# degleris1/CMF.jl

Measured on AMD Instinct MI355X. Metric: MU iters/sec (convolutive NMF multiplicative update; achieved HBM GB/s in `hbm`), higher is better.
Workload: dtype f32

## Files before the change

### cmf.jl_amd/csrc/cmf_api.hip

```cpp
#include "cmf_internal.h"

static void wb_free(cmf_handle_s *h);
static void wb_disarm(cmf_handle_s *h);

size_t n_partial(const cmf_handle_s *h)
{
    const CmfDims &d = h->d;
    size_t n = (size_t)(64 * h->conv_gx) * (size_t)std::max(h->conv_gy, h->conv_gy_ext);
    n = std::max(n, (size_t)(d.Np / 64) * d.KB * d.L);
    n = std::max(n, (size_t)((d.Tl + 63) / 64) * d.KB);
    n = std::max(n, 2 * (((size_t)d.Tl * d.K32 + 1023) / 1024));
    return n;
}

static int ensure_stage(cmf_handle_s *h, size_t elems)
{
    if (h->stage_elems >= elems) return CMF_OK;
    if (h->stage) HIPCHK(hipFree(h->stage));
    h->stage = nullptr;
    h->stage_elems = 0;
    HIPCHK(hipMalloc(&h->stage, elems * sizeof(double)));
    h->stage_elems = elems;
    return CMF_OK;
}
// ... 354 lines not shown
    const CmfDims &d = h->d;
    h->spec_gen = -1;
    HxtParams p;
    p.H = h->H; p.X0 = X0; p.X1 = X1; p.slabs = slabs;
    p.Np = NpX; p.K32 = d.K32; p.KB = d.KB; p.PADL = d.PADL; p.L = d.L; p.Tl = main_rows >= 0 ? main_rows : d.Tl; p.chunk_len = chunk_len;
    p.G = h->hxt_groups; p.nsrc = nsrc;
    p.CG = hxt_cg(nchunks);
    dim3 grid((NpX / 128) * p.CG * h->hxt_groups, nchunks / p.CG, nsrc * d.KB), block(256);
    switch (h->hxt_LP) {
#define CASE(LP_) case LP_: hipLaunchKernelGGL((hxt_kernel<LP_>), grid, block, 0, h->stream, p); break;
        CASE(1) CASE(2) CASE(3) CASE(4) CASE(5) CASE(6) CASE(8)
#undef CASE
    default: return fail(CMF_ERR_STATE, "internal: bad hxt LP %d", h->hxt_LP);
    }
    for (int i = 0; i < 7; ++i)
        if (kHxtLP[i] == h->hxt_LP) h->launches[LA_HXT + i] += 1;
    h->launches[nsrc == 1 ? LA_HXT_NSRC1 : LA_HXT_NSRC2] += 1;
    h->launches[p.Tl < d.Tl ? LA_HXT_TAIL : LA_HXT_NO_TAIL] += 1;
    KCHK("hxt_kernel");
    return CMF_OK;
}

static int launch_hxt(cmf_handle_s *h)
{
    return launch_hxt_on(h, h->X, h->est, h->d.Np, 2, h->wslabs, h->hxt_nchunks, h->hxt_chunk_len, h->hxt_main);
}

int launch_transconv(cmf_handle_s *h, int nsrc, const float *xt0, bool front_block)
{
    if (h->sk_tc) return launch_transconv_small(h, nsrc, xt0);
    ProfScope prof_(h, nsrc == 2 ? PROF_TRANSCONV : PROF_TRANSCONV_1);
    const CmfDims &d = h->d;
    TcParams p;
    p.Wn = h->Wn; p.XT0 = xt0 ? xt0 : h->XT; p.XT1 = h->estT; p.slabs = h->hslabs;
    p.NpW = d.Np;
    p.TP = d.TP; p.PADL = d.PADL; p.K32 = d.K32; p.KB = d.KB; p.L = d.L; p.Tl = d.Tl;
    p.nsrc = nsrc;
    p.C = (int)(rup(d.N, 8) / 8);
    p.W = nsrc == 2 ? h->tc_W : h->tc_W1;
    p.F = nsrc == 2 ? h->tc_S : h->tc_S1;
    p.wtab = h->tc_tab[nsrc == 2 ? 0 : 1];
    p.t_first = 0;
    p.slab_rows = d.Tl;
    if (front_block) {
        p.W = h->tc_W2; p.F = h->tc_S2; p.wtab = h->tc_tab[2];
        p.t_first = -128;
        p.slab_rows = d.Tl + 128;
    }
    dim3 grid((p.W + 3) / 4), block(256);
    switch (h->tc_LT) {
#define CASE(LT_) case LT_: hipLaunchKernelGGL((transconv_kernel<LT_>), grid, block, 0, h->stream, p); break;
        CASE(4) CASE(8) CASE(12) CASE(16) CASE(20) CASE(24) CASE(28) CASE(32)
#undef CASE
    default: return fail(CMF_ERR_STATE, "internal: bad transconv LT %d", h->tc_LT);
    }
    h->launches[LA_TC + h->tc_LT / 4 - 1] += 1;
    if (front_block) h->launches[LA_TC_FRONT] += 1;
    if (p.W >= 64 && p.W % 32 == 0) h->launches[LA_TC_XCD] += 1;
    KCHK("transconv_kernel");
    return CMF_OK;
}

int launch_slab_sum(cmf_handle_s *h, float *out, const float *in, int nslabs, size_t stride, bool take_carry,
                           CmfHxtTail tail)
{
    size_t n4 = stride / 4;
    int blocks = (int)std::min<size_t>(2048, (n4 + 255) / 256);
    CmfLossCarry carry{};
    if (take_carry && h->carry.partial) {
        carry = h->carry;
        h->carry = CmfLossCarry{};
    }
    hipLaunchKernelGGL(slab_sum_kernel, dim3(blocks + (carry.partial ? 1 : 0)), dim3(256), 0, h->stream, out, in, nslabs, stride, n4, carry, tail);
    h->launches[carry.partial ? LA_SLAB_SUM_CARRY : LA_SLAB_SUM] += 1;
    KCHK("slab_sum_kernel");
    return CMF_OK;
}

int hxt_contract(cmf_handle_s *h, const float *X0, const float *X1, int nsrc, float *out, bool take_carry, bool slabs_only)
{
    const CmfDims &d = h->d;
    h->spec_gen = -1;
    if (h->small_k) return hxt_contract_small(h, X0, X1, nsrc, out, take_carry, slabs_only);
    const int nch = nsrc == 2 ? h->hxt_nchunks : h->hxt_nchunks1, clen = nsrc == 2 ? h->hxt_chunk_len : h->hxt_chunk_len1;
    const int main_rows = nsrc == 2 ? h->hxt_main : h->hxt_main1;
    CMFTRY(launch_hxt_on(h, X0, X1, d.Np, nsrc, h->wslabs, nch, clen, main_rows));
    const CmfHxtTail tail{h->H, X0, X1, d.Tl - main_rows, d.PADL + main_rows, d.L, d.K32, d.Np};
    return launch_slab_sum(h, out, h->wslabs, hxt_nslabs(nch), (size_t)nsrc * d.L * d.K32 * d.Np, take_carry, tail);
}

int read_scalar(cmf_handle_s *h, int slot, double *v)
{
    HIPCHK(hipMemcpyAsync(h->h_scalar + slot, h->d_scalar + slot, sizeof(double), hipMemcpyDeviceToHost, h->stream));
    HIPCHK(hipStreamSynchronize(h->stream));
    *v = h->h_scalar[slot];
    return CMF_OK;
}

static int check_ready(cmf_handle_s *h, bool need_data)
{
    if (!h) return fail(CMF_ERR_ARG, "handle is NULL");
    if (h->root_only) return fail(CMF_ERR_STATE, "this entry needs a single-GPU handle, not the front handle of a cmf_create_multi group");
    HIPCHK(hipSetDevice(h->device));
    if (!h->factors_set) return fail(CMF_ERR_STATE, "factors not set: call cmf_set_factors first");
    if (need_data && !h->have_data) return fail(CMF_ERR_STATE, "handle was created without data");
    return CMF_OK;
}

static bool w_speculated(cmf_handle_s *h)
{
    const bool hit = h->spec_gen >= 0 && h->spec_gen == h->est_gen && h->reuse_est && h->est_kind == mu_est_kind(h) && !h->carry.partial;
    h->spec_gen = -1;
    if (hit) h->spec_hits += 1;
    return hit;
}

static int mu_conv_est(cmf_handle_s *h)
{
    return h->mu_mask ? launch_conv<8>(h, h->est, h->d.Tl, h->conv_gy) : launch_conv<0>(h, h->est, h->d.Tl, h->conv_gy);
}

int w_partial_impl(cmf_handle_s *h)
{
    const CmfDims &d = h->d;
    if (w_speculated(h)) return CMF_OK;
    if (!(h->reuse_est && h->est_kind == mu_est_kind(h)))
        CMFTRY(mu_conv_est(h));
    set_est(h, mu_est_kind(h));
    return hxt_contract(h, mu_X(h), h->est, 2, h->numden, true);
}

int w_partial_half_impl(cmf_handle_s *h, int den)
{
    const CmfDims &d = h->d;
    const size_t LKN = (size_t)d.L * d.K32 * d.Np;
    if (den) {
        if (!(h->reuse_est && h->est_kind == 1))
            CMFTRY(launch_conv<0>(h, h->est, d.Tl, h->conv_gy));
        set_est(h, 1);
    }
    const float *src = den ? h->est : h->X;
    return hxt_contract(h, src, src, 1, h->numden + (den ? LKN : 0), den != 0);
}

static int w_apply_impl_(cmf_handle_s *h, double l1W, double l2W, const float *tail_src, float *tail_dst, int tail_n, const float *den);
int w_apply_impl(cmf_handle_s *h, double l1W, double l2W, const float *tail_src, float *tail_dst, int tail_n,
                        const float *den)
{
    return w_apply_impl_(h, l1W, l2W, tail_src, tail_dst, tail_n, den);
}

static int kl_w_phase_impl(cmf_handle_s *h, double l1W, double l2W)
{
    const CmfDims &d = h->d;
    if (h->mu_mask) {
        if (!(h->reuse_est && h->est_kind == 8)) CMFTRY(launch_conv<12>(h, h->est, d.Tl, h->conv_gy, h->Xm));
        set_est(h, 8);
        CMFTRY(hxt_contract(h, h->est, h->M, 2, h->numden, true));
        return w_apply_impl(h, l1W, l2W, nullptr, nullptr, 0, nullptr);
    }
    if (!(h->reuse_est && h->est_kind == 7)) CMFTRY(launch_conv<12>(h, h->est, d.Tl, h->conv_gy));
    set_est(h, 7);
    CMFTRY(hxt_contract(h, h->est, h->est, 1, h->numden, true));
    float *den = h->numden + (size_t)d.L * d.K32 * d.Np;
    hipLaunchKernelGGL(kl_hsum_kernel, dim3(d.K, KL_HCHUNKS), dim3(256), 0, h->stream, h->Ht, d.TP, d.PADL, d.Tl, h->kl_sums);
    KCHK("kl_hsum_kernel");
    hipLaunchKernelGGL(kl_den_w_kernel, dim3(d.L, d.K), dim3(256), 0, h->stream, h->Ht, h->kl_sums, den, d.TP, d.PADL, d.Tl, d.K32, d.Np);
    KCHK("kl_den_w_kernel");
    return w_apply_impl(h, l1W, l2W, nullptr, nullptr, 0, den);
}

static int kl_h_update_impl(cmf_handle_s *h, double l1H, double l2H)
{
    const CmfDims &d = h->d;
    if (h->mu_mask) {
        CMFTRY(launch_conv<13>(h, h->estT, d.Tl + h->halo_r, h->conv_gy_ext, h->XmT));
        CMFTRY(launch_transconv(h, 2, h->MT));
        const size_t TKm = (size_t)d.Tl * d.K32;
        hipLaunchKernelGGL(h_update_kernel, dim3((d.Tl + HUPD_T - 1) / HUPD_T, d.KB), dim3(256), 0, h->stream, h->H, h->Ht, h->hslabs + TKm, 2 * TKm, h->tc_S,
                           h->hslabs, 2 * TKm, h->tc_S, d.Tl, d.K, d.K32, d.PADL, d.TP, (float)l1H, (float)(2.0 * l2H));
        KCHK("h_update_kernel");
        set_est(h, 0);
        return wb_after_H(h);
    }
    CMFTRY(launch_conv<13>(h, h->estT, d.Tl + h->halo_r, h->conv_gy_ext));
    CMFTRY(launch_transconv(h, 1, h->estT));
    hipLaunchKernelGGL(kl_wsum_kernel, dim3(d.L, d.K), dim3(256), 0, h->stream, h->Wt, d.K32, d.Np, h->kl_sums);
    KCHK("kl_wsum_kernel");
    const size_t TK = (size_t)d.Tl * d.K32;
    hipLaunchKernelGGL(kl_den_h_kernel, dim3((unsigned)((TK + 255) / 256)), dim3(256), 0, h->stream, h->kl_sums, h->kl_denH, d.Tl, d.K, d.K32, d.L);
    KCHK("kl_den_h_kernel");
    hipLaunchKernelGGL(h_update_kernel, dim3((d.Tl + HUPD_T - 1) / HUPD_T, d.KB), dim3(256), 0, h->stream, h->H, h->Ht, h->hslabs, TK, h->tc_S1,
                       h->kl_denH, (size_t)0, 1, d.Tl, d.K, d.K32, d.PADL, d.TP, (float)l1H, (float)(2.0 * l2H));
    KCHK("h_update_kernel");
    set_est(h, 0);
    return wb_after_H(h);
}

static int w_phase_impl(cmf_handle_s *h, double l1W, double l2W)
{
    const CmfDims &d = h->d;
    if (h->mu_div) return kl_w_phase_impl(h, l1W, l2W);
    if (!h->small_k) {
        CMFTRY(w_partial_impl(h));
        return w_apply_impl(h, l1W, l2W);
    }
    if (!w_speculated(h)) {
        if (!(h->reuse_est && h->est_kind == mu_est_kind(h)))
            CMFTRY(mu_conv_est(h));
        set_est(h, mu_est_kind(h));
        CMFTRY(hxt_contract(h, mu_X(h), h->est, 2, nullptr, false, true));
    }
    CmfLossCarry carry{};
    if (h->carry.partial) {
        carry = h->carry;
        h->carry = CmfLossCarry{};
    }
    hipLaunchKernelGGL(w_update_small_kernel, dim3(d.Np / 64 + 1, d.L, d.K), dim3(256), 0, h->stream, h->Wt, h->Wn, h->sk_tc ? h->sk_Wj : nullptr, h->sk_slabs,
                       h->sk_ngroups, d.N, d.K, d.L, d.Np, d.K32, h->sk_JP, h->sk3_Kg, h->sk3_GR, h->sk3_JP,
                       (float)l1W, (float)(2.0 * l2W), carry);
    KCHK("w_update_small_kernel");
    set_est(h, 0);
    h->sk_wj_gen = h->sk_tc ? h->est_gen : -1;
    return CMF_OK;
}

static int w_apply_impl_(cmf_handle_s *h, double l1W, double l2W, const float *tail_src, float *tail_dst, int tail_n, const float *den)
{
    const CmfDims &d = h->d;
    dim3 grid(d.Np / 64, d.KB, d.L);
    if (!den) den = h->numden + (size_t)d.L * d.K32 * d.Np;
    hipLaunchKernelGGL(w_update_kernel, grid, dim3(256), 0, h->stream, h->Wt, h->Wn, h->numden, den,
                       d.N, d.K, d.L, d.Np, d.K32, (float)l1W, (float)(2.0 * l2W), tail_src, tail_dst, tail_n);
    KCHK("w_update_kernel");
    set_est(h, 0);
    return CMF_OK;
}

int h_update_impl(cmf_handle_s *h, double l1H, double l2H, bool front)
{
    const CmfDims &d = h->d;
    if (front) {
        if (!h->halo_ext || !h->left_data) return fail(CMF_ERR_STATE, "internal: this shard cannot update the columns in front of its own");
        int np = 0;
        CMFTRY(launch_conv_rows<1>(h, h->estT, -1, 1 + (d.Tl + h->halo_r + 63) / 64, 0, h->n_cu, nullptr, nullptr, nullptr, &np, d.Tl + h->halo_r));
        CMFTRY(launch_transconv(h, 2, nullptr, true));
        const int hx = h->halo_ext, R = d.Tl + 128;
        dim3 gridx((d.Tl + hx + HUPD_T - 1) / HUPD_T, d.KB);
        const float *num = h->hslabs + (size_t)(128 - hx) * d.K32;
        hipLaunchKernelGGL(h_update_kernel, gridx, dim3(256), 0, h->stream, h->H, h->Ht, num, (size_t)2 * R * d.K32, h->tc_S2, num + (size_t)R * d.K32,
                           (size_t)2 * R * d.K32, h->tc_S2, d.Tl + hx, d.K, d.K32, d.PADL - hx, d.TP, (float)l1H, (float)(2.0 * l2H));
        KCHK("h_update_kernel");
        set_est(h, 0);
        return wb_after_H(h);
    }
    if (h->mu_div) return kl_h_update_impl(h, l1H, l2H);
    if (h->mu_mask) CMFTRY(launch_conv<9>(h, h->estT, d.Tl + h->halo_r, h->conv_gy_ext));
    else CMFTRY(launch_conv<1>(h, h->estT, d.Tl + h->halo_r, h->conv_gy_ext));
    if (sk_can_fuse_h(h)) {
        CMFTRY(launch_transconv_small(h, 2, mu_XT(h), true, (float)l1H, (float)(2.0 * l2H)));
        ++h->sk_fused_h;
        set_est(h, 0);
        return wb_after_H(h);
    }
    CMFTRY(launch_transconv(h, 2, mu_XT(h)));
    dim3 grid((d.Tl + HUPD_T - 1) / HUPD_T, d.KB);
    const size_t TK = (size_t)d.Tl * d.K32;
    hipLaunchKernelGGL(h_update_kernel, grid, dim3(256), 0, h->stream, h->H, h->Ht, h->hslabs, 2 * TK, h->tc_S, h->hslabs + TK, 2 * TK, h->tc_S,
                       d.Tl, d.K, d.K32, d.PADL, d.TP, (float)l1H, (float)(2.0 * l2H));
    KCHK("h_update_kernel");
    set_est(h, 0);
    return wb_after_H(h);
}

int launch_loss_conv(cmf_handle_s *h)
{
    const CmfDims &d = h->d;
    if (h->mu_div && h->mu_mask) {
        if (!h->reuse_est) return launch_conv<18>(h, nullptr, d.Tl, h->conv_gy, h->Xm);
        CMFTRY(launch_conv<19>(h, h->est, d.Tl, h->conv_gy, h->Xm));
        set_est(h, 8);
        return CMF_OK;
    }
    if (h->mu_div) {
        if (!h->reuse_est) return launch_conv<14>(h, nullptr, d.Tl, h->conv_gy);
        CMFTRY(launch_conv<15>(h, h->est, d.Tl, h->conv_gy));
        set_est(h, 7);
        return CMF_OK;
    }
    if (h->mu_mask) {
        if (!h->reuse_est) return launch_conv<10>(h, nullptr, d.Tl, h->conv_gy);
        CMFTRY(launch_conv<11>(h, h->est, d.Tl, h->conv_gy));
        set_est(h, 6);
        return CMF_OK;
    }
    if (h->reuse_est && !h->gram) {
        CMFTRY(launch_conv<3>(h, h->est, d.Tl, h->conv_gy));
        set_est(h, 1);
        return CMF_OK;
    }
    return launch_conv<2>(h, nullptr, d.Tl, h->conv_gy);
}

static int w_speculate(cmf_handle_s *h)
{
    if (!(h->reuse_est && h->est_kind == mu_est_kind(h)) || h->gram || h->group || h->carry.partial || h->mu_div) return CMF_OK;
    if (h->small_k) CMFTRY(hxt_contract(h, mu_X(h), h->est, 2, nullptr, false, true));
    else CMFTRY(hxt_contract(h, mu_X(h), h->est, 2, h->numden, true));
    h->spec_gen = h->est_gen;
    return CMF_OK;
}

static int ensure_ring(cmf_handle_s *h)
{
    if (!h->h_ring) HIPCHK(hipHostMalloc(&h->h_ring, 3 * sizeof(double), hipHostMallocCoherent));
    return CMF_OK;
}


int loss_partial_impl(cmf_handle_s *h, double *sumsq, bool readback, double *host_out, bool speculate)
{
    volatile unsigned long long *word = nullptr;
    if (readback && !host_out) {
        CMFTRY(ensure_ring(h));
        host_out = h->h_ring + 2;
        word = reinterpret_cast<volatile unsigned long long *>(host_out);
        *word = CMF_SENTINEL64;
    }
    CMFTRY(launch_loss_conv(h));
    hipLaunchKernelGGL(loss_reduce_kernel, dim3(1), dim3(256), 0, h->stream, h->partial, h->conv_partials, h->d_scalar, host_out);
    KCHK("loss_reduce_kernel");
    if (speculate) CMFTRY(w_speculate(h));
    if (!readback) return CMF_OK;
    if (!word) return read_scalar(h, 0, sumsq);
    CMFTRY(wait_words<unsigned long long>(h->stream, word, 1, CMF_SENTINEL64, nullptr, nullptr));
    *sumsq = h->h_ring[2];
    return CMF_OK;
}

int set_factors_impl(cmf_handle_s *h, const double *W, const double *H)
{
    if (!h || (!W && !H)) return fail(CMF_ERR_ARG, "NULL argument");
    if ((!W || !H) && !h->factors_set) return fail(CMF_ERR_STATE, "the first cmf_set_factors needs both W and H");
    HIPCHK(hipSetDevice(h->device));
    const CmfDims &d = h->d;
    const size_t nW = (size_t)d.L * d.N * d.K, nH = (size_t)d.Tl * d.K;
    CMFTRY(ensure_stage(h, std::max(nW, nH)));
    if (W) {
        HIPCHK(hipMemsetAsync(h->Wt, 0, (size_t)d.Lp * d.K32 * d.Np * sizeof(float), h->stream));
        HIPCHK(hipMemsetAsync(h->Wn, 0, (size_t)d.Lp * d.Np * d.K32 * sizeof(float), h->stream));
        HIPCHK(hipMemcpyAsync(h->stage, W, nW * sizeof(double), hipMemcpyHostToDevice, h->stream));
        hipLaunchKernelGGL(pack_W_kernel, dim3(1024), dim3(256), 0, h->stream, h->stage, d.N, d.K, d.L, h->Wt, h->Wn, d.Np, d.K32);
        KCHK("pack_W_kernel");
        HIPCHK(hipStreamSynchronize(h->stream));
    }
    if (H) {
        HIPCHK(hipMemsetAsync(h->H, 0, (size_t)d.TP * d.K32 * sizeof(float), h->stream));
        HIPCHK(hipMemsetAsync(h->Ht, 0, (size_t)d.K32 * d.TP * sizeof(float), h->stream));
        HIPCHK(hipMemcpyAsync(h->stage, H, nH * sizeof(double), hipMemcpyHostToDevice, h->stream));
        hipLaunchKernelGGL(pack_H_kernel, dim3(1024), dim3(256), 0, h->stream, h->stage, d.Tl, d.K, h->H, h->Ht, d.K32, d.TP, d.PADL);
        KCHK("pack_H_kernel");
        HIPCHK(hipStreamSynchronize(h->stream));
    }
    h->factors_set = true;
    set_est(h, 0);
    return CMF_OK;
}

int get_factors_impl(cmf_handle_s *h, double *W, double *H)
{
    if (!h) return fail(CMF_ERR_ARG, "handle is NULL");
    CMFTRY(check_ready(h, false));
    const CmfDims &d = h->d;
    const size_t nW = (size_t)d.L * d.N * d.K, nH = (size_t)d.Tl * d.K;
    CMFTRY(ensure_stage(h, std::max(nW, nH)));
    if (W) {
        hipLaunchKernelGGL(unpack_W_kernel<double>, dim3(1024), dim3(256), 0, h->stream, h->stage, d.N, d.K, d.L, h->Wn, d.Np, d.K32);
        KCHK("unpack_W_kernel");
        HIPCHK(hipMemcpyAsync(W, h->stage, nW * sizeof(double), hipMemcpyDeviceToHost, h->stream));
        HIPCHK(hipStreamSynchronize(h->stream));
    }
    if (H) {
        hipLaunchKernelGGL(unpack_H_kernel<double>, dim3(1024), dim3(256), 0, h->stream, h->stage, d.Tl, d.K, h->H, d.K32, d.PADL);
        KCHK("unpack_H_kernel");
        HIPCHK(hipMemcpyAsync(H, h->stage, nH * sizeof(double), hipMemcpyDeviceToHost, h->stream));
        HIPCHK(hipStreamSynchronize(h->stream));
    }
    return CMF_OK;
}

// ... 309 lines not shown
        return cmf_create_multi(h, R, devs.data(), CMF_COMM_LOOPBACK, N, T, K, L, data);
    }
    return create_impl(h, device, N, T, K, L, data, 0, T, false);
}

int cmf_create_shard(cmf_handle *h, int device, int64_t N, int64_t T_local, int64_t K, int64_t L,
                     const double *data_local, int64_t t_offset, int64_t T_global)
{
    if (!data_local) return fail(CMF_ERR_ARG, "data_local is NULL");
    if (T_local < L - 1 && T_local != T_global)
        return fail(CMF_ERR_UNSUPPORTED, "a shard must hold at least L-1 = %lld columns (got %lld)", (long long)(L - 1), (long long)T_local);
    return create_impl(h, device, N, T_local, K, L, data_local, t_offset, T_global, true);
}

int cmf_shard_set_left_data(cmf_handle h, const double *cols)
{
    if (!h || !cols) return fail(CMF_ERR_ARG, "NULL argument");
    if (h->group) return fail(CMF_ERR_STATE, "call cmf_shard_set_left_data before the shard joins its group (cmf_comm_init_*)");
    if (!h->sharded) return fail(CMF_ERR_STATE, "cmf_shard_set_left_data needs a handle from cmf_create_shard");
    if (!h->halo_ext) return CMF_OK;
    HIPCHK(hipSetDevice(h->device));
    CMFTRY(upload_cols(h, cols, -h->halo_ext, h->halo_ext, false, false));
    h->left_data = true;
    return CMF_OK;
}

int cmf_destroy(cmf_handle h)
{
    if (h && h->group) {
        cmf_group_s *g = h->group;
        if (h->wb && !h->wb->pool.empty()) {
            for (cmf_handle_s *s : g->sh)
                if (s->wb) s->wb->cancel.store(true, std::memory_order_release);
            if (!cmf_pool_wait(h->wb->pool, 5.0))
                return fail(CMF_ERR_HIP, "cmf_destroy: a write-back helper is stuck in a device wait; the group was not freed");
        }
        std::vector<cmf_handle_s *> shards = g->sh;
        if (!group_destroy(g))
            return fail(CMF_ERR_COMM, "cmf_destroy: an enqueue worker is stuck inside a call that does not return; the group and its shards were not freed");
        for (cmf_handle_s *s : shards) {
            s->group = nullptr;
            if (s != h) destroy_impl(s);
        }
        h->group = nullptr;
    }
    destroy_impl(h);
    return CMF_OK;
}

int cmf_synchronize(cmf_handle h)
{
    if (!h) return fail(CMF_ERR_ARG, "handle is NULL");
    if (h->group) return group_sync(h->group);
    HIPCHK(hipSetDevice(h->device));
    HIPCHK(hipStreamSynchronize(h->stream));
    return CMF_OK;
}

int cmf_rccl_version(int *version, char *path, int64_t path_len)
{
    if (!version) return fail(CMF_ERR_ARG, "version is NULL");
    CMFTRY(rccl_load());
    RCCLCHK(g_rccl.GetVersion(version));
    if (path && path_len > 0) snprintf(path, (size_t)path_len, "%s", g_rccl.path.c_str());
    return CMF_OK;
}

int cmf_get_counter(cmf_handle h, const char *name, int64_t *value)
{
    if (!h || !name || !value) return fail(CMF_ERR_ARG, "NULL argument");
    if (std::strcmp(name, "hals_pipeline_reruns") == 0) { *value = h->hals_reruns; return CMF_OK; }
    if (std::strcmp(name, "writeback_calls") == 0) { *value = h->wb ? h->wb->armed_calls : 0; return CMF_OK; }
    if (std::strcmp(name, "speculated_contractions") == 0) { *value = h->spec_hits; return CMF_OK; }
    if (std::strcmp(name, "liveness_checks") == 0) { *value = g_liveness_checks.load(); return CMF_OK; }
    if (admm_counter(h, name, value)) return CMF_OK;
    if (sep_counter(h, name, value)) return CMF_OK;
    if (anls_counter(h, name, value)) return CMF_OK;
    if (std::strcmp(name, "small_k_fused_h_updates") == 0) {
        *value = h->sk_fused_h;
        if (h->group)
            for (const cmf_handle_s *s : h->group->sh) *value += (s != h) ? s->sk_fused_h : 0;
        return CMF_OK;
    }
    if (std::strcmp(name, "writeback_overlapped") == 0) { *value = h->wb ? h->wb->hooked_calls : 0; return CMF_OK; }
    if (std::strncmp(name, "launches:", 9) == 0) {
        for (int c = 0; c < LA_NCLS; ++c)
            if (std::strcmp(name + 9, kLaunchNames[c]) == 0) {
                *value = h->launches[c];
                if (h->group)
                    for (const cmf_handle_s *s : h->group->sh) *value += (s != h) ? s->launches[c] : 0;
                return CMF_OK;
            }
        return fail(CMF_ERR_ARG, "unknown launch path '%s'", name + 9);
    }
    if (h->group) {
        cmf_group_s *g = h->group;
        if (std::strcmp(name, "allreduce_calls") == 0) { *value = g->n_allreduce; return CMF_OK; }
        if (std::strcmp(name, "allgather_calls") == 0) { *value = g->n_allgather; return CMF_OK; }
        if (std::strcmp(name, "halo_in_allreduce") == 0) { *value = (g->halo_opt && g->halo_can && !g->gram && g->nranks > 1) ? 1 : 0; return CMF_OK; }
        if (std::strcmp(name, "enqueue_ns") == 0) { *value = g->enqueue_ns; return CMF_OK; }
        if (std::strcmp(name, "enqueue_iters") == 0) { *value = g->enqueue_iters; return CMF_OK; }
        if (std::strcmp(name, "worker_ns") == 0) {
            int64_t m = 0;
            for (const auto &w : g->pool.w) m = std::max<int64_t>(m, w->busy_ns.load());
            *value = m;
            return CMF_OK;
        }
    }
    return fail(CMF_ERR_ARG, "unknown counter '%s'", name);
}

int cmf_set_stream(cmf_handle h, void *hip_stream)
{
    if (!h) return fail(CMF_ERR_ARG, "handle is NULL");
    if (h->group) return fail(CMF_ERR_STATE, "a group handle runs on its own per-device streams");
    if ((hipStream_t)hip_stream != h->stream) {
        HIPCHK(hipSetDevice(h->device));
        HIPCHK(hipStreamSynchronize(h->stream));
        h->spec_gen = -1;
        h->hals_spec_gen = -1;
    }
    h->stream = (hipStream_t)hip_stream;
    return CMF_OK;
}

static const char *const kOptionNames[] = {"reuse_est", "speculate", "gram", "conv_kernel", "conv_split", "small_k", "small_k_fuse", "hals_prepare", "hals_gram",
                                           "hals_persist", "hals_general", "hals_seg", "hals_lag", "hals_debug", "hals_chase", "profile", "profile_mask",
                                           "allreduce_overlap", "enqueue_threads", "halo_in_allreduce"};
int cmf_option_names(char *buf, int64_t len)
{
    if (!buf || len < 1) return fail(CMF_ERR_ARG, "bad buffer");
    std::string all;
    for (const char *n : kOptionNames) all += (all.empty() ? "" : ",") + std::string(n);
    if ((int64_t)all.size() + 1 > len) return fail(CMF_ERR_ARG, "buffer too small: %zu bytes needed", all.size() + 1);
    std::memcpy(buf, all.c_str(), all.size() + 1);
    return CMF_OK;
}

int cmf_set_option(cmf_handle h, const char *name, int value)
{
    if (!h || !name) return fail(CMF_ERR_ARG, "NULL argument");
    if (std::strcmp(name, "anls_backup_only") == 0) {
        if (h->group || h->root_only || h->sharded) return fail(CMF_ERR_UNSUPPORTED, "anls_backup_only: the ANLS rule runs on single-GPU handles only");
        if (value != 0 && value != 1) return fail(CMF_ERR_ARG, "anls_backup_only must be 0 or 1");
        h->anls_backup_only = value;
        return CMF_OK;
    }
    if (std::strcmp(name, "nnls_large") == 0) {
        if (h->group || h->root_only || h->sharded) return fail(CMF_ERR_UNSUPPORTED, "nnls_large: the ANLS rule and the separable fit run on single-GPU handles only");
        if (value != 0 && value != 1) return fail(CMF_ERR_ARG, "nnls_large must be 0 or 1");
        h->nnls_large = value;
        return CMF_OK;
    }
    if (std::strcmp(name, "kl_mask") == 0) {
        if (h->group || h->root_only || h->sharded) return fail(CMF_ERR_UNSUPPORTED, "kl_mask: the mask and the divergence of the MU rule are chosen on single-GPU handles only");
        if (value != 0 && value != 1) return fail(CMF_ERR_ARG, "kl_mask must be 0 or 1");
        if (!value && h->mu_mask && h->mu_div) return fail(CMF_ERR_STATE, "kl_mask: the KL form and a mask are both installed; clear the mask or restore CMF_DIV_SQUARE first");
        h->kl_mask = value;
        return CMF_OK;
    }
    if (h->group) {
        cmf_group_s *g = h->group;
        CMFTRY(group_join(g));
        if (std::strcmp(name, "allreduce_overlap") == 0) {
            CMFTRY(group_sync(g));
            if (value) CMFTRY(group_ensure_lane1(g));
            g->overlap = value != 0;
            g->num_ready = false;
            return CMF_OK;
        }
        if (std::strcmp(name, "halo_in_allreduce") == 0) {
            CMFTRY(group_sync(g));
            g->halo_opt = value != 0;
            g->halos_current = false;
            g->halos_pending = false;
            g->halo_wide = false;
            g->num_ready = false;
            return CMF_OK;
        }
        if (std::strcmp(name, "enqueue_threads") == 0) {
            CMFTRY(group_sync(g));
            if (value) return group_start_workers(g);
            (void)group_stop_workers(g);
            return CMF_OK;
        }
        if (std::strcmp(name, "gram") == 0) {
            if (value != 0 && value != 1) return fail(CMF_ERR_UNSUPPORTED, "sharded handles take gram = 0 or 1 (the loss of gram = 2 is not exact to 1e-4)");
            if (value && g->nranks > 1 && g->T < 4 * g->L)
                return fail(CMF_ERR_UNSUPPORTED, "the Gram form on a sharded handle needs T >= 4 L (got T=%lld, L=%lld)", (long long)g->T, (long long)g->L);
            CMFTRY(group_sync(g));
            for (size_t i = 0; i < g->sh.size(); ++i) {
                cmf_handle_s *s = g->sh[i];
                CMFTRY(group_use(s));
                if (value) CMFTRY(gram_ensure(s));
                if (value && i < g->red.size() && g->red[i])
                    HIPCHK(hipMemsetAsync(g->red[i] + g->LKN2 / 2, 0, (size_t)g->HHsz * sizeof(float), s->stream));
                s->gram = value;
                set_est(s, 0);
                s->carry = CmfLossCarry{};
            }
            g->gram = value;
            g->num_ready = false;
            return CMF_OK;
        }
        for (cmf_handle_s *s : g->sh) {
            cmf_group_s *keep = s->group;
            s->group = nullptr;
            const int rc = cmf_set_option(s, name, value);
            s->group = keep;
            if (rc != CMF_OK) return rc;
        }
        g->num_ready = false;
        return CMF_OK;
    }
    if (std::strcmp(name, "allreduce_overlap") == 0 || std::strcmp(name, "enqueue_threads") == 0 || std::strcmp(name, "halo_in_allreduce") == 0) return CMF_OK;
    if (std::strcmp(name, "gram") == 0) {
        if (value < 0 || value > 2) return fail(CMF_ERR_ARG, "gram must be 0, 1 or 2");
        if (value && h->sharded && h->T_global != h->d.Tl) return fail(CMF_ERR_STATE, "the Gram form is not available on sharded handles");
        if (value && h->mu_div) return fail(CMF_ERR_UNSUPPORTED, "the Gram forms rewrite the squared-error denominators and have no KL form: "
                                                                 "restore CMF_DIV_SQUARE with cmf_mu_set_divergence first");
        if (value && h->mu_mask) return fail(CMF_ERR_UNSUPPORTED, "the Gram forms have no masked form (the Gram rewriting of the denominators needs mask .* est, "
                                                                  "which is not a product of Gram matrices): clear the mask of cmf_mu_set_mask first");
        h->gram = value;
        set_est(h, 0);
        return CMF_OK;
    }
    if (std::strcmp(name, "conv_kernel") == 0) {
        if (value != 0 && value != 2 && value != 3) return fail(CMF_ERR_ARG, "conv_kernel must be 0 (per mode), 2 or 3");
        h->conv_variant = value;
        set_est(h, 0);
        return CMF_OK;
    }
    if (std::strcmp(name, "hals_gram") == 0) {
        h->hals_gram = (value == 1 || value == 2) ? value : 0;
// ... 1081 lines not shown
```

### cmf.jl_amd/csrc/cmf_internal.h

```cpp
#pragma once
#pragma GCC visibility push(default)
#include "cmf_hip.h"
#pragma GCC visibility pop
#include "cmf_kernels.h"
#include "cmf_rng.h"
#include "cmf_writeback.h"

#include <algorithm>
#include <atomic>
#include <chrono>
#include <cmath>
#include <cstdarg>
#include <cstdio>
#include <cstring>
#include <functional>
#include <map>
#include <mutex>
#include <string>
#include <thread>
#include <vector>

inline thread_local std::string g_err;

static int fail(int code, const char *fmt, ...)
// ... 83 lines not shown
    }
    ~RoctxRange()
    {
        if (on) roctx_api().pop();
    }
};

enum { LA_CONV = 0, LA_CONV2, LA_CONV3_WHOLE, LA_CONV3_WHOLE_P4, LA_CONV3_WHOLE_P16, LA_CONV3_P4, LA_CONV3_P16,
       LA_CONV_SMALL,  LA_CONV_SMALL_Q = LA_CONV_SMALL + 6, LA_CONV_SMALL_PRE,
       LA_HXT,  LA_HXT_NSRC1 = LA_HXT + 7, LA_HXT_NSRC2, LA_HXT_TAIL, LA_HXT_NO_TAIL,
       LA_TC,  LA_TC_FRONT = LA_TC + 8, LA_TC_XCD,
       LA_HXT_SMALL,  LA_HXT_SMALL_RV = LA_HXT_SMALL + 10,
       LA_GFOLD = LA_HXT_SMALL_RV + 3,  LA_GFOLD_RV = LA_GFOLD + 6,  LA_GFOLD_SPLIT = LA_GFOLD_RV + 3, LA_GFOLD_FUSED_H,
       LA_GRAM_W, LA_GRAM_CORR, LA_GRAM_TAPS, LA_GRAM_H_MFMA, LA_GRAM_H,
       LA_SLAB_SUM, LA_SLAB_SUM_CARRY, LA_SLAB_SUM_SMALL, LA_SLAB_SUM_SMALL_CARRY,
       LA_HALO_PACK2, LA_HALO_UNPACK2, LA_HALO_PACK3, LA_HALO_UNPACK3, LA_NCLS };
static const char *const kLaunchNames[] = {
    "conv_kernel", "conv2_kernel", "conv3_kernel:whole", "conv3_kernel:whole+4", "conv3_kernel:whole+16", "conv3_kernel:pieces4", "conv3_kernel:pieces16",
    "conv_small_kernel<1>", "conv_small_kernel<2>", "conv_small_kernel<3>", "conv_small_kernel<4>", "conv_small_kernel<6>", "conv_small_kernel<8>",
    "conv_small_kernel:quarter", "conv_small_kernel:pre",
    "hxt_kernel<1>", "hxt_kernel<2>", "hxt_kernel<3>", "hxt_kernel<4>", "hxt_kernel<5>", "hxt_kernel<6>", "hxt_kernel<8>",
    "hxt_kernel:nsrc1", "hxt_kernel:nsrc2", "hxt_kernel:tail", "hxt_kernel:no_tail",
    "transconv_kernel<4>", "transconv_kernel<8>", "transconv_kernel<12>", "transconv_kernel<16>", "transconv_kernel<20>", "transconv_kernel<24>",
    "transconv_kernel<28>", "transconv_kernel<32>", "transconv_kernel:front_block", "transconv_kernel:xcd",
    "hxt_small_kernel<1>", "hxt_small_kernel<2>", "hxt_small_kernel<3>", "hxt_small_kernel<4>", "hxt_small_kernel<5>", "hxt_small_kernel<6>",
    "hxt_small_kernel<7>", "hxt_small_kernel<8>", "hxt_small_kernel<9>", "hxt_small_kernel<10>",
    "hxt_small_kernel<1,RV>", "hxt_small_kernel<2,RV>", "hxt_small_kernel<3,RV>",
    "g_gemm_fold_small_kernel<1>", "g_gemm_fold_small_kernel<2>", "g_gemm_fold_small_kernel<3>", "g_gemm_fold_small_kernel<4>",
    "g_gemm_fold_small_kernel<5>", "g_gemm_fold_small_kernel<6>",
    "g_gemm_fold_small_kernel<1,RV>", "g_gemm_fold_small_kernel<2,RV>", "g_gemm_fold_small_kernel<3,RV>",
    "g_gemm_fold_small_kernel:split", "g_gemm_fold_small_kernel:fused_h",
    "gram_w_kernel", "gram_lag_corr", "gram_w_taps", "gram_h_mfma_kernel", "gram_h_kernel",
    "slab_sum_kernel", "slab_sum_kernel:carry", "slab_sum_small_kernel", "slab_sum_small_kernel:carry",
    "halo_pack2_kernel", "halo_unpack2_kernel", "halo_pack3_kernel", "halo_unpack3_kernel"};
static_assert(sizeof(kLaunchNames) / sizeof(kLaunchNames[0]) == LA_NCLS, "one name per launch path");

struct cmf_handle_s {
    int device = 0;
    CmfDims d{};
    int64_t t_offset = 0, T_global = 0;
    int halo_r = 0;
    bool has_left = false;
    bool sharded = false;

    hipStream_t own_stream = nullptr, stream = nullptr;
    hipEvent_t ev0 = nullptr, ev1 = nullptr;

    float *H = nullptr, *Ht = nullptr, *Wt = nullptr, *Wn = nullptr;
    float *X = nullptr, *XT = nullptr, *est = nullptr, *estT = nullptr;
    float *wslabs = nullptr;
    float *numden = nullptr;
    float *numden_own = nullptr;
    float *hslabs = nullptr;
    float *halo[4] = {nullptr, nullptr, nullptr, nullptr};
    float *halo_own[4] = {nullptr, nullptr, nullptr, nullptr};
    double *partial = nullptr;
    double *d_scalar = nullptr;
    double *d_scalar_own = nullptr;
    double *h_scalar = nullptr;
    double *stage = nullptr;
    size_t stage_elems = 0;

    int hxt_LP = 1, hxt_groups = 1, hxt_nchunks = 1, hxt_chunk_len = 2;
    int tc_LT = 4, tc_S = 1, tc_W = 4;
    int tc_S1 = 1, tc_W1 = 4;
    int tc_S2 = 1, tc_W2 = 4;
    int halo_ext = 0;
    bool left_data = false;
    std::vector<int4> tc_tab_host[3];
    int4 *tc_tab[3] = {nullptr, nullptr, nullptr};
    int hxt_nchunks1 = 1, hxt_chunk_len1 = 6;
    int hxt_main = 0, hxt_main1 = 0;
    bool small_k = false;
    bool small_k_ok = false;
    bool sk_tc_ok = false, sk_tc = false;
    int sk_J = 0, sk_JP = 0, sk_MG = 1, sk_MBW = 4, sk_chunk_len = 16, sk_ngroups = 1, sk_TG = 128;
    int sk_RV = 0;
    int sk3_MG = 1, sk3_MBW = 4, sk3_Kg = 1, sk3_JP = 128;
    int sk3_NS = 1, sk3_RPS = 1;
    int sk3_GR = 128, sk3_RV = 0;
    float *sk_slabs = nullptr, *sk_Wj = nullptr;
    int *sk_cnt = nullptr;
    int64_t sk_fused_h = 0;
    int sk_fuse = 1;
    int64_t sk_wj_gen = -1;
    int tc_S_full = 1, tc_S1_full = 1;
    int conv_gx = 1, conv_gy = 1, conv_gy_ext = 1;
    int conv_variant = 0;
    int conv_partials = 1;
    int conv_split = 1;
    int n_cu = 256;

    bool hals_ready = false;
    bool gram_ready = false;
    int hals_NpH = 0, hals_NpC = 0, hals_TPp = 0, hals_ne = 0, hals_t_edge0 = 0, hals_corr_R = 4;
    float *hals_HX = nullptr, *hals_cslabs = nullptr, *hals_C = nullptr, *hals_HH = nullptr, *hals_PT = nullptr, *hals_D = nullptr;
    float *hals_PW = nullptr, *hals_GW = nullptr, *hals_GE = nullptr, *hals_GWt = nullptr;
    int hals_seg = 256, hals_nseg = 1;
    int hals_gram = 2;
    bool hals_w_general = false, hals_h_general = false;
    int hals_opt_persist = 1, hals_opt_general = 0, hals_opt_seg = 384, hals_opt_lag = 2, hals_debug = 0;
    int hals_opt_chase = -1;
    hipStream_t hals_sA = nullptr, hals_sB = nullptr;
    hipEvent_t hals_ev[3] = {nullptr, nullptr, nullptr};
    int hals_mask_aper = 0;
    int hals_cuB = 0;
    int hals_chased_rows = 0, hals_chased_partials = 0;
    int hals_pullers = 0;
    int *hals_flags = nullptr;
    int *hals_status = nullptr;
    float *hals_snap = nullptr;
    double hals_l1 = 0.0, hals_l2 = 0.0;
    int64_t hals_reruns = 0;

    double pgd_stepW = 5.0, pgd_stepH = 5.0, pgd_cur_loss = -1.0;
    float *pgd_gradH = nullptr;
    int mask_complement_now = 0;
    int pgd_loss_abs_now = 0;
    int pgd_loss_abs = 0;
    double *pgd_knorm = nullptr;
    float *M = nullptr, *MT = nullptr;
    bool mu_mask = false;
    float *Xm = nullptr, *XmT = nullptr;
    double xm_sumsq = 0.0, xm_norm = 0.0;
    int mu_div = 0;
    double data_sum = 0.0;
    int kl_mask = 0;
    float *kl_denH = nullptr;
    double *kl_sums = nullptr;

    double data_sumsq = 0.0, data_norm = 0.0;
    bool factors_set = false;
    bool have_data = false;
    bool reuse_est = true;
    int gram = 0;
    float *gram_numden_h = nullptr;
    bool prof = false;
    int prof_every = 1;
    int prof_seen[32] = {0};
    int64_t launches[LA_NCLS] = {0};
    struct ProfRec { hipEvent_t a, b; int cls; };
    unsigned prof_mask = 0;
    std::vector<ProfRec> prof_recs;
    std::vector<hipEvent_t> prof_pool;
    int est_kind = 0;
    void *arena = nullptr;
    size_t arena_bytes = 0;
    bool streams_may_hang = false;
    int64_t est_gen = 0;
    int64_t spec_gen = -1;
    int last_rule_call = 0;
    bool speculate = true;
    std::function<int()> after_reduce;
    int64_t hals_spec_gen = -1;
    int64_t spec_hits = 0;

    struct cmf_group_s *group = nullptr;
    bool root_only = false;
    hipStream_t own_comm_stream = nullptr, comm_stream = nullptr;
    hipEvent_t ev_c0 = nullptr, ev_c1 = nullptr;
    double *h_ring = nullptr;
    bool dev_stamps = false;
    CmfLossCarry carry{};
    CmfWriteback *wb = nullptr;
    struct AdmmState *admm = nullptr;
    struct AnlsState *anls = nullptr;
// ... 414 lines not shown
```

### cmf.jl_amd/csrc/cmf_kernels.h

```cpp
#pragma once
#include <hip/hip_runtime.h>
#include <type_traits>
#include <stdint.h>

typedef float f32x16 __attribute__((ext_vector_type(16)));
typedef float f32x4 __attribute__((ext_vector_type(4)));

#define CMF_EPS_F 2.220446049250313e-16f

struct CmfDims {
    int N, Tl, K, L;
    int Np;
    int KB;
    int K32;
    int PADL;
    int TP;
    int Lp;
};

__device__ __forceinline__ int cmf_crow(int r, int h) { return (r & 3) + 8 * (r >> 2) + 4 * h; }

__device__ __forceinline__ __amdgpu_buffer_rsrc_t cmf_rsrc(const void *base, size_t bytes)
{
    return __builtin_amdgcn_make_buffer_rsrc(const_cast<void *>(base), 0,
// ... 1381 lines not shown
    return ((s[0] + s[1]) + (s[2] + s[3])) + ((s[4] + s[5]) + (s[6] + s[7]));
}

struct CmfLossCarry {
    const double *partial;
    int n;
    double *out;
    double *host_out;
    float *tail;
    int tail_len, rank;
};

__device__ __forceinline__ void cmf_block_loss_reduce(const CmfLossCarry &c)
{
    __shared__ double red[256];
    red[threadIdx.x] = cmf_thread_loss_sum(c.partial, c.n);
    __syncthreads();
    for (int off = 128; off > 0; off >>= 1) {
        if ((int)threadIdx.x < off) red[threadIdx.x] += red[threadIdx.x + off];
        __syncthreads();
    }
    const double tot = red[0];
    if (threadIdx.x == 0) {
        *c.out = tot;
        if (c.host_out) __hip_atomic_store(c.host_out, tot, __ATOMIC_RELAXED, __HIP_MEMORY_SCOPE_SYSTEM);
    }
    if (c.tail) {
        const float hi = (float)tot, lo = (float)(tot - (double)hi);
        for (int j = threadIdx.x; j < c.tail_len; j += 256) c.tail[j] = (j == 2 * c.rank) ? hi : (j == 2 * c.rank + 1) ? lo : 0.f;
    }
}

struct CmfHxtTail {
    const float *H, *X0, *X1;
    int rows, t0, L, K32, Np;
};

static __global__ __launch_bounds__(256) void slab_sum_kernel(float *out, const float *in, int nslabs, size_t stride, size_t n4, CmfLossCarry carry,
                                                        CmfHxtTail tail)
{
    unsigned bx = blockIdx.x, nbx = gridDim.x;
    if (carry.partial) {
        if (bx == 0) { cmf_block_loss_reduce(carry); return; }
        --bx; --nbx;
    }
    for (size_t idx = bx * (size_t)blockDim.x + threadIdx.x; idx < n4; idx += (size_t)nbx * blockDim.x) {
        float4 a = reinterpret_cast<const float4 *>(in)[idx];
        for (int s = 1; s < nslabs; s += 4) {
            float4 b[4];
#pragma unroll
            for (int u = 0; u < 4; ++u) {
                const int su = (s + u < nslabs) ? s + u : s;
                b[u] = reinterpret_cast<const float4 *>(in + (size_t)su * stride)[idx];
            }
#pragma unroll
            for (int u = 0; u < 4; ++u)
                if (s + u < nslabs) { a.x += b[u].x; a.y += b[u].y; a.z += b[u].z; a.w += b[u].w; }
        }
        if (tail.rows > 0) {
            const size_t e = 4 * idx;
            const int n = (int)(e % tail.Np);
            const int k = (int)((e / tail.Np) % tail.K32);
            const int l = (int)((e / ((size_t)tail.Np * tail.K32)) % tail.L);
            const int src = (int)(e / ((size_t)tail.Np * tail.K32 * tail.L));
            const float *X = src ? tail.X1 : tail.X0;
            for (int r0 = 0; r0 < tail.rows; r0 += 6) {
                float hv[6];
                float4 xv[6];
#pragma unroll
                for (int u = 0; u < 6; ++u) {
                    const int t = tail.t0 + ((r0 + u < tail.rows) ? r0 + u : r0);
                    hv[u] = tail.H[(size_t)(t - l) * tail.K32 + k];
                    xv[u] = *reinterpret_cast<const float4 *>(X + (size_t)t * tail.Np + n);
                }
#pragma unroll
                for (int u = 0; u < 6; ++u)
                    if (r0 + u < tail.rows) {
                        a.x = fmaf(hv[u], xv[u].x, a.x); a.y = fmaf(hv[u], xv[u].y, a.y);
                        a.z = fmaf(hv[u], xv[u].z, a.z); a.w = fmaf(hv[u], xv[u].w, a.w);
                    }
            }
        }
        reinterpret_cast<float4 *>(out)[idx] = a;
    }
}

#define CMF_SENTINEL64 0xFFFFFFFFFFFFFFFFull
#define CMF_SENTINEL32 0xFFFFFFFFu
static __global__ __launch_bounds__(256) void loss_reduce_kernel(const double *partial, int n, double *out, double *host_out = nullptr)
{
    __shared__ double red[256];
    red[threadIdx.x] = cmf_thread_loss_sum(partial, n);
    __syncthreads();
    for (int off = 128; off > 0; off >>= 1) {
        if ((int)threadIdx.x < off) red[threadIdx.x] += red[threadIdx.x + off];
        __syncthreads();
    }
    if (threadIdx.x == 0) {
        *out = red[0];
        if (host_out) __hip_atomic_store(host_out, red[0], __ATOMIC_RELAXED, __HIP_MEMORY_SCOPE_SYSTEM);
    }
}



#define HALS_CORR_LPW 5
static __global__ __launch_bounds__(256) void hals_corr_kernel(const float *H, float *slabs, int K32, int KB, int PADL, int Tl, int L, int R)
{
    extern __shared__ float hc_rows[];
    const int tid = threadIdx.x;
    const int lane = tid & 63, wave = __builtin_amdgcn_readfirstlane(tid >> 6);
    const int i = lane & 31, h = lane >> 5;
    const int ab = blockIdx.y / KB, bb = blockIdx.y % KB;
    const int t_begin = blockIdx.x * R, t_end = (t_begin + R < Tl) ? t_begin + R : Tl;
    float *slab = slabs + (size_t)blockIdx.x * L * K32 * K32;
    {
        const f32x4 *src = reinterpret_cast<const f32x4 *>(H + (size_t)(PADL + t_begin - (L - 1)) * K32);
        f32x4 *dst = reinterpret_cast<f32x4 *>(hc_rows);
        const int nlive = (t_end - t_begin + L - 1) * K32 / 4, nall = (R + L - 1 + 4) * K32 / 4;
        for (int e = tid; e < nall; e += 256) dst[e] = e < nlive ? src[e] : f32x4{0.f, 0.f, 0.f, 0.f};
    }
    __syncthreads();
    const float *Hs = hc_rows + (size_t)(L - 1) * K32;
    const int nsteps = (t_end - t_begin + 3) / 4;
    for (int d0 = wave; d0 < L; d0 += 4 * HALS_CORR_LPW) {
        f32x16 acc[HALS_CORR_LPW];
#pragma unroll
        for (int q = 0; q < HALS_CORR_LPW; ++q)
#pragma unroll
            for (int r = 0; r < 16; ++r) acc[q][r] = 0.f;
        const float *pb = Hs + h * K32 + bb * 32 + i;
        const float *pa[HALS_CORR_LPW];
#pragma unroll
        for (int q = 0; q < HALS_CORR_LPW; ++q) pa[q] = Hs + (h - ((d0 + 4 * q < L) ? d0 + 4 * q : 0)) * K32 + ab * 32 + i;
        float a0[HALS_CORR_LPW], a1[HALS_CORR_LPW], b0 = pb[0], b1;
#pragma unroll
        for (int q = 0; q < HALS_CORR_LPW; ++q) a0[q] = pa[q][0];
        for (int s = 0; s < nsteps; ++s) {
            const int o = s * 4 * K32;
            b1 = pb[o + 2 * K32];
#pragma unroll
            for (int q = 0; q < HALS_CORR_LPW; ++q) a1[q] = pa[q][o + 2 * K32];
#pragma unroll
            for (int q = 0; q < HALS_CORR_LPW; ++q) acc[q] = __builtin_amdgcn_mfma_f32_32x32x2f32(a0[q], b0, acc[q], 0, 0, 0);
            b0 = pb[o + 4 * K32];
#pragma unroll
            for (int q = 0; q < HALS_CORR_LPW; ++q) a0[q] = pa[q][o + 4 * K32];
#pragma unroll
            for (int q = 0; q < HALS_CORR_LPW; ++q) acc[q] = __builtin_amdgcn_mfma_f32_32x32x2f32(a1[q], b1, acc[q], 0, 0, 0);
        }
#pragma unroll
        for (int q = 0; q < HALS_CORR_LPW; ++q) {
            const int d = d0 + 4 * q;
            if (d < L)
#pragma unroll
                for (int r = 0; r < 16; ++r) slab[((size_t)d * K32 + ab * 32 + cmf_crow(r, h)) * K32 + bb * 32 + i] = acc[q][r];
        }
    }
}
static __global__ __launch_bounds__(1024) void hals_corr_sum_kernel(const float *slabs, float *C, int G, int L, int K32, int NpC)
{
    __shared__ float part[16][64];
    const int lane = threadIdx.x & 63, wave = threadIdx.x >> 6;
    const size_t n = (size_t)L * K32 * K32, idx = (size_t)blockIdx.x * 64 + lane;
    float s = 0.f;
    if (idx < n)
// ... 1744 lines not shown
```

Measured before the change: 187.5.

## Fuse HXT slab reduction and tail into W update kernel

For the non-small-K MU path, the W phase now stops after the HXt contraction writes per-chunk slabs, and a new w_update_slabs_kernel does the rest in one pass. It sums the slabs, adds the tail rows, applies the multiplicative update, writes both W layouts and folds in the pending loss carry reduction. This removes the separate slab_sum launch and the numden intermediate write and read. In exchange the update kernel's grid does the slab reads serially per thread. It is enabled by default through a new option.

```diff
diff --git a/cmf.jl_amd/csrc/cmf_api.hip b/cmf.jl_amd/csrc/cmf_api.hip
--- a/cmf.jl_amd/csrc/cmf_api.hip
+++ b/cmf.jl_amd/csrc/cmf_api.hip
@@ -460,6 +460,9 @@
     const CmfDims &d = h->d;
     h->spec_gen = -1;
     if (h->small_k) return hxt_contract_small(h, X0, X1, nsrc, out, take_carry, slabs_only);
+    if (slabs_only)
+        return launch_hxt_on(h, X0, X1, d.Np, nsrc, h->wslabs, nsrc == 2 ? h->hxt_nchunks : h->hxt_nchunks1, nsrc == 2 ? h->hxt_chunk_len : h->hxt_chunk_len1,
+                             nsrc == 2 ? h->hxt_main : h->hxt_main1);
     const int nch = nsrc == 2 ? h->hxt_nchunks : h->hxt_nchunks1, clen = nsrc == 2 ? h->hxt_chunk_len : h->hxt_chunk_len1;
     const int main_rows = nsrc == 2 ? h->hxt_main : h->hxt_main1;
     CMFTRY(launch_hxt_on(h, X0, X1, d.Np, nsrc, h->wslabs, nch, clen, main_rows));
@@ -579,7 +582,7 @@
 {
     const CmfDims &d = h->d;
     if (h->mu_div) return kl_w_phase_impl(h, l1W, l2W);
-    if (!h->small_k) {
+    if (!h->small_k && !h->w_slabs) {
         CMFTRY(w_partial_impl(h));
         return w_apply_impl(h, l1W, l2W);
     }
@@ -593,6 +596,15 @@
     if (h->carry.partial) {
         carry = h->carry;
         h->carry = CmfLossCarry{};
+    }
+    if (!h->small_k) {
+        const CmfHxtTail tail{h->H, mu_X(h), h->est, d.Tl - h->hxt_main, d.PADL + h->hxt_main, d.L, d.K32, d.Np};
+        hipLaunchKernelGGL(w_update_slabs_kernel, dim3(d.Np / 64 + (carry.partial ? 1 : 0), d.KB, d.L), dim3(256), 0, h->stream, h->Wt, h->Wn, h->wslabs,
+                           hxt_nslabs(h->hxt_nchunks), d.N, d.K, d.L, d.Np, d.K32, (float)l1W, (float)(2.0 * l2W), carry, tail);
+        KCHK("w_update_slabs_kernel");
+        ++h->w_slabs_launches;
+        set_est(h, 0);
+        return CMF_OK;
     }
     hipLaunchKernelGGL(w_update_small_kernel, dim3(d.Np / 64 + 1, d.L, d.K), dim3(256), 0, h->stream, h->Wt, h->Wn, h->sk_tc ? h->sk_Wj : nullptr, h->sk_slabs,
                        h->sk_ngroups, d.N, d.K, d.L, d.Np, d.K32, h->sk_JP, h->sk3_Kg, h->sk3_GR, h->sk3_JP,
@@ -683,7 +695,7 @@
 static int w_speculate(cmf_handle_s *h)
 {
     if (!(h->reuse_est && h->est_kind == mu_est_kind(h)) || h->gram || h->group || h->carry.partial || h->mu_div) return CMF_OK;
-    if (h->small_k) CMFTRY(hxt_contract(h, mu_X(h), h->est, 2, nullptr, false, true));
+    if (h->small_k || h->w_slabs) CMFTRY(hxt_contract(h, mu_X(h), h->est, 2, nullptr, false, true));
     else CMFTRY(hxt_contract(h, mu_X(h), h->est, 2, h->numden, true));
     h->spec_gen = h->est_gen;
     return CMF_OK;
@@ -1159,6 +1171,7 @@
             for (const cmf_handle_s *s : h->group->sh) *value += (s != h) ? s->sk_fused_h : 0;
         return CMF_OK;
     }
+    if (std::strcmp(name, "w_update_slabs_launches") == 0) { *value = h->w_slabs_launches; return CMF_OK; }
     if (std::strcmp(name, "writeback_overlapped") == 0) { *value = h->wb ? h->wb->hooked_calls : 0; return CMF_OK; }
     if (std::strncmp(name, "launches:", 9) == 0) {
         for (int c = 0; c < LA_NCLS; ++c)
@@ -1227,6 +1240,12 @@
         if (h->group || h->root_only || h->sharded) return fail(CMF_ERR_UNSUPPORTED, "nnls_large: the ANLS rule and the separable fit run on single-GPU handles only");
         if (value != 0 && value != 1) return fail(CMF_ERR_ARG, "nnls_large must be 0 or 1");
         h->nnls_large = value;
+        return CMF_OK;
+    }
+    if (std::strcmp(name, "w_update_slabs") == 0) {
+        if (value != 0 && value != 1) return fail(CMF_ERR_ARG, "w_update_slabs must be 0 or 1");
+        h->w_slabs = value;
+        h->spec_gen = -1;
         return CMF_OK;
     }
     if (std::strcmp(name, "kl_mask") == 0) {
diff --git a/cmf.jl_amd/csrc/cmf_internal.h b/cmf.jl_amd/csrc/cmf_internal.h
--- a/cmf.jl_amd/csrc/cmf_internal.h
+++ b/cmf.jl_amd/csrc/cmf_internal.h
@@ -189,6 +189,8 @@
     float *sk_slabs = nullptr, *sk_Wj = nullptr;
     int *sk_cnt = nullptr;
     int64_t sk_fused_h = 0;
+    int w_slabs = 1;
+    int64_t w_slabs_launches = 0;
     int sk_fuse = 1;
     int64_t sk_wj_gen = -1;
     int tc_S_full = 1, tc_S1_full = 1;
diff --git a/cmf.jl_amd/csrc/cmf_kernels.h b/cmf.jl_amd/csrc/cmf_kernels.h
--- a/cmf.jl_amd/csrc/cmf_kernels.h
+++ b/cmf.jl_amd/csrc/cmf_kernels.h
@@ -1487,6 +1487,84 @@
             }
         }
         reinterpret_cast<float4 *>(out)[idx] = a;
+    }
+}
+
+static __global__ __launch_bounds__(256) void w_update_slabs_kernel(float *Wt, float *Wn, const float *slabs, int nslabs, int N, int K, int L, int Np,
+                                                              int K32, float l1, float two_l2, CmfLossCarry carry, CmfHxtTail tail)
+{
+    __shared__ float tile[32][65];
+    if ((int)blockIdx.x == Np / 64) {
+        if (blockIdx.y == 0 && blockIdx.z == 0) cmf_block_loss_reduce(carry);
+        return;
+    }
+    const int tid = threadIdx.x;
+    const int n0 = blockIdx.x * 64, kb = blockIdx.y, l = blockIdx.z;
+    const int nn = tid & 63, n = n0 + nn;
+    const size_t LKN = (size_t)L * K32 * Np;
+    {
+        size_t idx[8];
+        float w[8], num[8], den[8];
+#pragma unroll
+        for (int q = 0; q < 8; ++q) {
+            idx[q] = ((size_t)l * K32 + kb * 32 + q * 4 + (tid >> 6)) * Np + n;
+            w[q] = Wt[idx[q]];
+            num[q] = slabs[idx[q]];
+            den[q] = slabs[LKN + idx[q]];
+        }
+        for (int s = 1; s < nslabs; ++s) {
+            const float *sl = slabs + (size_t)s * 2 * LKN;
+            float a[8], b[8];
+#pragma unroll
+            for (int q = 0; q < 8; ++q) {
+                a[q] = sl[idx[q]];
+                b[q] = sl[LKN + idx[q]];
+            }
+#pragma unroll
+            for (int q = 0; q < 8; ++q) {
+                num[q] += a[q];
+                den[q] += b[q];
+            }
+        }
+        if (tail.rows > 0) {
+            const float *hb = tail.H + kb * 32 + (tid >> 6);
+            for (int r0 = 0; r0 < tail.rows; r0 += 2) {
+                float hv[2][8], x0[2], x1[2];
+#pragma unroll
+                for (int u = 0; u < 2; ++u) {
+                    const int t = tail.t0 + ((r0 + u < tail.rows) ? r0 + u : r0);
+                    x0[u] = tail.X0[(size_t)t * Np + n];
+                    x1[u] = tail.X1[(size_t)t * Np + n];
+#pragma unroll
+                    for (int q = 0; q < 8; ++q) hv[u][q] = hb[(size_t)(t - l) * K32 + q * 4];
+                }
+#pragma unroll
+                for (int u = 0; u < 2; ++u)
+                    if (r0 + u < tail.rows) {
+#pragma unroll
+                        for (int q = 0; q < 8; ++q) {
+                            num[q] = fmaf(hv[u][q], x0[u], num[q]);
+                            den[q] = fmaf(hv[u][q], x1[u], den[q]);
+                        }
+                    }
+            }
+        }
+#pragma unroll
+        for (int q = 0; q < 8; ++q) {
+            const int kk = q * 4 + (tid >> 6), k = kb * 32 + kk;
+            const float wn = (k < K && n < N) ? cmf_mu(w[q], num[q], den[q], l1, two_l2) : 0.f;
+            Wt[idx[q]] = wn;
+            tile[kk][nn] = wn;
+        }
+    }
+    __syncthreads();
+    {
+        const int kk = tid & 31;
+#pragma unroll
+        for (int q = 0; q < 8; ++q) {
+            const int n2 = q * 8 + (tid >> 5);
+            Wn[((size_t)l * Np + n0 + n2) * K32 + kb * 32 + kk] = tile[kk][n2];
+        }
     }
 }
 
```

Result: no change. 188.0 (median of 6 runs) (+0.2%).
